# evanmayer/effex

Hardware: AMD Instinct MI355X
Metric: 2-ant FX correlator throughput (PFB+FFT+X, integrated) (higher is better)
Workload: dtype f32; 1 GPU; configs[1]: 2-antenna FX, num_samp=262144, ntaps=4, nchan=4096, 10000 integration frames per GPU per step; frames_per_gpu=10000, frames_total=10000, resident_frames=10000, num_samp=262144, nchan=4096, ntaps=4, n_ant=2, sample_definition=one complex sample per antenna stream, reduce_transport=none (single rank), library=effex_amd/csrc/libfxcorr.so

## Files before the change

effex_amd/csrc/fx_fused4096.h:

```cpp
#pragma once
#include "fx_math.h"

#if defined(__HIP_DEVICE_COMPILE__)
#define FXC_SCHED_FENCE() __builtin_amdgcn_sched_barrier(0)
#else
#define FXC_SCHED_FENCE() ((void)0)
#endif

namespace fxc {
namespace fused {

FX_HD cf lds_load(const cf* p) {
#if defined(__HIP_DEVICE_COMPILE__)
    typedef const volatile __attribute__((address_space(3))) unsigned long long* lds_u64_ptr;
    const unsigned long long u = *(lds_u64_ptr)(p);
    cf r;
    r.x = __uint_as_float((unsigned)(u & 0xffffffffull));
    r.y = __uint_as_float((unsigned)(u >> 32));
    return r;
#else
    return *p;
#endif
}

constexpr int kN = 4096;
constexpr int kT = 4;
constexpr int kThreads = 512;
constexpr int kRowPitch = 272;
constexpr int kRegion = 16 * kRowPitch;
constexpr int kAccPerThread = 8;
#ifndef FXC_FIR_GROUP
#define FXC_FIR_GROUP 4
#endif
constexpr int kFirGroup = FXC_FIR_GROUP;

constexpr int kLdsWin = 0;
constexpr int kLdsRegion = kLdsWin + kN * 16;
constexpr int kLdsTw2 = kLdsRegion + 2 * kRegion * 8;
constexpr int kLdsBytes = kLdsTw2 + 256 * 8;

struct State {
    cf h[4][16];
    cf tw1[16];
    cf acc[kAccPerThread];
};

template <int PH>
FX_HD void state_reset_history(State& s) {
#pragma unroll
    for (int d = 1; d < 4; ++d)
#pragma unroll
        for (int r = 0; r < 16; ++r) s.h[(PH + d) & 3][r] = mk(0.f, 0.f);
}

FX_HD void state_reset_all(State& s) {
    state_reset_history<0>(s);
#pragma unroll
    for (int q = 0; q < kAccPerThread; ++q) s.acc[q] = mk(0.f, 0.f);
}

struct RangeWalk {
    int c, i;
    int left;
    int row;
    int n_pts;
    int seg, seg_left;
    int seg_jump;
    int unit, in_row;
    int row_step;
    int row_off;
    bool rows_are_chunks;
    bool lead;
};

struct RangeSplit {
    int rounds, n_full, n_tail, rows_rounds, n_rows;
};

FX_HD RangeSplit range_split(int g, int n_chunks, int seg, int unit, bool rows_are_chunks) {
    RangeSplit r;
    r.rounds = n_chunks / (g * seg);
    r.n_full = r.rounds * g * seg;
    r.n_tail = n_chunks - r.n_full;
    r.rows_rounds = rows_are_chunks ? r.n_full : g * ((r.rounds * seg + unit - 1) / unit);
    r.n_rows = r.rows_rounds + r.n_tail + g;
    return r;
}

FX_HD RangeWalk range_walk_rounds(int b, int g, int n_chunks, int n_pts, int seg,
                                   int unit, bool rows_are_chunks) {
    const RangeSplit sp = range_split(g, n_chunks, seg, unit, rows_are_chunks);
    RangeWalk w;
    w.c = b * seg;
    w.i = 0;
    w.left = sp.rounds * seg * n_pts;
    w.n_pts = n_pts;
    w.seg = w.seg_left = seg;
    w.seg_jump = (g - 1) * seg;
    w.unit = rows_are_chunks ? 1 : unit;
    w.in_row = 0;
    w.rows_are_chunks = rows_are_chunks;
    w.row_off = 0;
    w.row_step = g;
    w.row = rows_are_chunks ? w.c : b;
    w.lead = false;
    return w;
}

FX_HD RangeWalk range_walk_tail(int b, int g, int n_chunks, int n_pts, int seg,
                                 int unit, bool rows_are_chunks) {
    const RangeSplit sp = range_split(g, n_chunks, seg, unit, rows_are_chunks);
    RangeWalk w;
    const int n_frames = sp.n_tail * n_pts;
    const int f0 = range_begin(b, n_frames, g);
    w.left = range_begin(b + 1, n_frames, g) - f0;
    w.c = sp.n_full + f0 / n_pts;
    w.i = f0 % n_pts;
    w.n_pts = n_pts;
    w.seg = 1;
    w.seg_left = 1;
    w.seg_jump = 0;
    w.unit = 1;
    w.in_row = 0;
    w.rows_are_chunks = true;
    w.row_off = sp.rows_rounds - sp.n_full;
    w.row_step = 0;
    w.lead = w.i != 0;
    w.row = w.lead ? sp.rows_rounds + sp.n_tail + b : w.c + w.row_off;
    return w;
}

FX_HD bool range_walk_row_ends(const RangeWalk& w) {
    return w.left == 1 || (w.i + 1 == w.n_pts && w.in_row + 1 == w.unit);
}

FX_HD void range_walk_prefetch(const RangeWalk& w, int& pc, int& pi) {
    pc = w.c;
    pi = w.i;
    if (w.left > 1 && ++pi == w.n_pts) {
        pi = 0;
        pc += 1 + (w.seg_left == 1 ? w.seg_jump : 0);
    }
}

FX_HD void range_walk_advance(RangeWalk& w, bool row_ended) {
    if (++w.i == w.n_pts) {
        w.i = 0;
        w.c += 1;
        if (--w.seg_left == 0) {
            w.c += w.seg_jump;
            w.seg_left = w.seg;
        }
        w.in_row += 1;
    }
    w.left -= 1;
    if (row_ended) {
        w.in_row = 0;
        w.row = w.rows_are_chunks ? w.c + w.row_off : w.row + w.row_step;
    }
}

FX_HD int sample_offset(int j, int r) { return (kN - 1) - j - 256 * r; }

template <int PH, int G = kFirGroup>
FX_HD void phase1_fir(const State& s, const f4* win, int tid, cf (&v)[16]) {
    const int j = tid & 255;
    const cf (&x0)[16] = s.h[PH];
    const cf (&x1)[16] = s.h[(PH + 3) & 3];
    const cf (&x2)[16] = s.h[(PH + 2) & 3];
    const cf (&x3)[16] = s.h[(PH + 1) & 3];
    constexpr int NG = 16 / G;
    f4 w[2][G];
#pragma unroll
    for (int q = 0; q < G; ++q) w[0][q] = win[q * 256 + j];
#pragma unroll
    for (int g = 0; g < NG; ++g) {
        if (g < NG - 1) {
#pragma unroll
            for (int q = 0; q < G; ++q) w[(g + 1) & 1][q] = win[(G * (g + 1) + q) * 256 + j];
        }
        FXC_SCHED_FENCE();
#pragma unroll
        for (int q = 0; q < G; ++q) {
            const int r = G * g + q;
            const f4 t = w[g & 1][q];
            cf a = cscale(x0[r], t.x);
            a = cfma(t.y, x1[r], a);
            a = cfma(t.z, x2[r], a);
            v[r] = cfma(t.w, x3[r], a);
        }
        FXC_SCHED_FENCE();
    }
}

FX_HD cf tw1_of(const cf (&pw2)[4], int k1) {
    cf w = mk(1.f, 0.f);
    bool have = false;
#pragma unroll
    for (int b = 0; b < 4; ++b) {
        if (k1 & (1 << b)) {
            w = have ? cmul(w, pw2[b]) : pw2[b];
            have = true;
        }
    }
    return w;
}

template <bool LEAN_TW = false>
FX_HD void phase1_finish_store(const State& s, cf (&v)[16], cf* region, int tid) {
    cf* mine = region + (tid >> 8) * kRegion + (tid & 255);
    cf pw2[4] = {s.tw1[1], s.tw1[2], s.tw1[4], s.tw1[8]};
#if defined(__HIP_DEVICE_COMPILE__)
    if (LEAN_TW) {
#pragma unroll
        for (int b = 0; b < 4; ++b) asm volatile("" : "+v"(pw2[b].x), "+v"(pw2[b].y));
    }
#endif
    dft16_b_stream(v, [&](int k1, cf val) {
        if (k1 > 0) val = cmul(val, LEAN_TW ? tw1_of(pw2, k1) : s.tw1[k1]);
        mine[k1 * kRowPitch] = val;
    });
}

FX_HD void state_load_twiddles(State& s, const cf* tw1_table, int tid) {
    const int j = tid & 255;
#pragma unroll
    for (int k1 = 0; k1 < 16; ++k1) s.tw1[k1] = tw1_table[k1 * 256 + j];
}

FX_HD cf* lane_row(cf* region, int tid) {
    const int l = tid & 63, wave = tid >> 6;
    const int ant = l >> 5, k1 = 2 * wave + ((l >> 4) & 1);
    return region + ant * kRegion + k1 * kRowPitch;
}

FX_HD void phase2_load(cf* region, int tid, cf (&v)[16]) {
    const cf* row = lane_row(region, tid);
    const int j0 = tid & 15;
#pragma unroll
    for (int j1 = 0; j1 < 16; ++j1) v[j1] = lds_load(row + j0 + 16 * j1);
}

FX_HD void phase2_twiddle(cf (&v)[16], const cf* tw2, int tid) {
    const int j0 = tid & 15;
    cf t[2][4];
#pragma unroll
    for (int q = 1; q < 4; ++q) t[0][q] = lds_load(tw2 + q * 16 + j0);
#pragma unroll
    for (int g = 0; g < 4; ++g) {
        if (g < 3) {
#pragma unroll
            for (int q = 0; q < 4; ++q) t[(g + 1) & 1][q] = lds_load(tw2 + (4 * (g + 1) + q) * 16 + j0);
        }
        FXC_SCHED_FENCE();
#pragma unroll
        for (int q = 0; q < 4; ++q) {
            const int q1 = 4 * g + q;
            if (q1 > 0) v[q1] = cmul(v[q1], t[g & 1][q]);
        }
        FXC_SCHED_FENCE();
    }
}

FX_HD void phase2_store(const cf (&v)[16], cf* region, int tid) {
    cf* row = lane_row(region, tid);
    const int j0 = tid & 15;
#pragma unroll
    for (int q1 = 0; q1 < 16; ++q1) row[q1 * 17 + j0] = v[q1];
}

FX_HD void phase3_load(cf* region, int tid, cf (&v)[16]) {
    const cf* row = lane_row(region, tid);
    const int q1 = tid & 15;
#pragma unroll
    for (int j0 = 0; j0 < 16; ++j0) v[j0] = lds_load(row + q1 * 17 + j0);
}

FX_HD void xacc(State& s, int q, cf a, cf b) { s.acc[q] = cmulc_acc(s.acc[q], a, b); }

FX_HD int bin_of(int tid, int q) {
    const int l = tid & 63, wave = tid >> 6;
    const int k1 = 2 * wave + ((l >> 4) & 1), q1 = l & 15, q2 = q + 8 * (l >> 5);
    return k1 + 16 * q1 + 256 * q2;
}

FX_HD int slot_of_bin(int k) {
    const int k1 = k & 15, q1 = (k >> 4) & 15, q2 = k >> 8;
    const int l = (q2 >> 3) * 32 + (k1 & 1) * 16 + q1;
    const int tid = (k1 >> 1) * 64 + l;
    return (q2 & 7) * kThreads + tid;
}

FX_HD int lane_specpos(int tid) {
    const int l = tid & 63, wave = tid >> 6;
    return (2 * wave + ((l >> 4) & 1)) * 16 + (l & 15);
}

FX_HD int specpos(int lane_l, int q2) { return (q2 >> 1) * 512 + 2 * lane_l + (q2 & 1); }
FX_HD int specpos_of_bin(int k) { return specpos((k & 15) * 16 + ((k >> 4) & 15), k >> 8); }

}
}
```

effex_amd/csrc/k_fused4096.h:

```cpp
#pragma once

namespace {

__device__ __forceinline__ void wave_sync() {
    __builtin_amdgcn_fence(__ATOMIC_RELEASE, "wavefront");
    __builtin_amdgcn_wave_barrier();
    __builtin_amdgcn_fence(__ATOMIC_ACQUIRE, "wavefront");
}

__device__ __forceinline__ void permlane32_swap(cf& a, cf& b) {
    auto rx = __builtin_amdgcn_permlane32_swap(__float_as_uint(a.x), __float_as_uint(b.x), false, false);
    auto ry = __builtin_amdgcn_permlane32_swap(__float_as_uint(a.y), __float_as_uint(b.y), false, false);
    a = fxc::mk(__uint_as_float(rx[0]), __uint_as_float(ry[0]));
    b = fxc::mk(__uint_as_float(rx[1]), __uint_as_float(ry[1]));
}

typedef unsigned v2u32 __attribute__((ext_vector_type(2)));
typedef unsigned v4u32 __attribute__((ext_vector_type(4)));
#ifndef FXC_LOAD_AUX_U8
#define FXC_LOAD_AUX_U8 2
#endif
#ifndef FXC_LOAD_AUX
#define FXC_LOAD_AUX 2
#endif
template <int R0, int CNT>
__device__ __forceinline__ void load_frame_part(cf (&xr)[16], const cf* chunk_base, unsigned chunk_bytes, unsigned voff,
                                                int64_t i) {
    __amdgpu_buffer_rsrc_t rs = __builtin_amdgcn_make_buffer_rsrc(const_cast<cf*>(chunk_base), 0, (int)chunk_bytes,
                                                                   0x00020000);
    const unsigned soff = (unsigned)(i * fxc::fused::kN * (int64_t)sizeof(cf));
#pragma unroll
    for (int r = R0; r < R0 + CNT; ++r) {
        const v2u32 d = __builtin_amdgcn_raw_buffer_load_b64(rs, voff, soff + (unsigned)(256 * (15 - r) * sizeof(cf)), FXC_LOAD_AUX);
        xr[r] = fxc::mk(__uint_as_float(d[0]), __uint_as_float(d[1]));
    }
}

template <int R0, int CNT>
__device__ __forceinline__ void load_frame_part_u8(cf (&xr)[16], const unsigned short* chunk_base,
                                                   unsigned chunk_bytes, unsigned voff, int64_t i) {
    __amdgpu_buffer_rsrc_t rs = __builtin_amdgcn_make_buffer_rsrc(const_cast<unsigned short*>(chunk_base), 0,
                                                                   (int)chunk_bytes, 0x00020000);
    const unsigned soff = (unsigned)(i * fxc::fused::kN * (int64_t)sizeof(unsigned short));
#pragma unroll
    for (int r = R0; r < R0 + CNT; ++r)
        xr[r].x = __uint_as_float(
            (unsigned)__builtin_amdgcn_raw_buffer_load_b16(rs, voff, soff + (unsigned)(256 * (15 - r) * sizeof(unsigned short)), FXC_LOAD_AUX_U8));
}

__device__ __forceinline__ void convert_frame_u8(cf (&h)[16], cf off) {
    const float k = 1.0f / 127.5f;
#pragma unroll
    for (int r = 0; r < 16; ++r) {
        const unsigned raw = __float_as_uint(h[r].x);
        h[r] = fxc::mk(fmaf((float)(raw & 0xFFu), k, off.x), fmaf((float)((raw >> 8) & 0xFFu), k, off.y));
    }
}

#ifndef FXC_ABL
#define FXC_ABL 0
#endif
#ifndef FXC_STAMPS
#define FXC_STAMPS 0
#endif
constexpr int kStampSegs = 12;
constexpr int kDckLdsBytes = 64;
constexpr int kAutoLdsBytes = fxc::fused::kAccPerThread * fxc::fused::kThreads * 4;
#if FXC_STAMPS
#define FXC_STAMP(k)                                                              \
    do {                                                                          \
        __builtin_amdgcn_sched_barrier(0);                                        \
        const unsigned long long t_now__ = __builtin_amdgcn_s_memtime();          \
        __builtin_amdgcn_s_waitcnt(0xC07F);                                       \
        seg[k] += t_now__ - t_prev;                                               \
        t_prev = t_now__;                                                         \
        __builtin_amdgcn_sched_barrier(0);                                        \
    } while (0)
#else
#define FXC_STAMP(k)
#endif
#if (FXC_ABL & 16)
#define FXC_PREFETCH(R0) ((void)0)
#else
#define FXC_PREFETCH(R0)                                                                                        \
    do {                                                                                                        \
        FXC_SCHED_FENCE();                                                                                      \
        if (U8)                                                                                                 \
            load_frame_part_u8<R0, 4>(nx, reinterpret_cast<const unsigned short*>(x) + (int64_t)pc * 2 * num_samp, \
                                      chunk_bytes, voff, nframe);                                               \
        else                                                                                                    \
            load_frame_part<R0, 4>(nx, nbase, chunk_bytes, voff, nframe);                                       \
        FXC_SCHED_FENCE();                                                                                      \
    } while (0)
#endif

struct U8State {
    cf off;
    bool have_next;
    bool rounds;
};

typedef unsigned v4u32_t __attribute__((ext_vector_type(4)));
constexpr int kDckStageVecs = 2 * fxc::fused::kThreads;

__device__ __forceinline__ void dck_fetch(const unsigned char* pair_base, int64_t num_samp, int64_t i, int tid, v4u32_t* stage) {
    typedef __attribute__((address_space(3))) v4u32_t* lptr_t;
    unsigned t = (unsigned)tid;
    asm volatile("" : "+v"(t));
    const unsigned lane_off = ((t >> 8) & 1u) * (unsigned)(2 * num_samp) + (t & 255u) * 16u;
    const unsigned char* base = pair_base + i * (fxc::fused::kThreads * 16);
    const unsigned lds_wave = __builtin_amdgcn_readfirstlane((unsigned)(size_t)(lptr_t)(stage + (t >> 6) * 128));
    unsigned m0_saved;
    asm volatile(
        "s_mov_b32 %[sv], m0\n\t"
        "s_mov_b32 m0, %[l0]\n\t"
        "s_nop 0\n\t"
        "global_load_lds_dwordx4 %[o0], %[base]\n\t"
        "s_add_u32 m0, %[l0], 0x400\n\t"
        "s_nop 0\n\t"
        "global_load_lds_dwordx4 %[o1], %[base]\n\t"
        "s_mov_b32 m0, %[sv]\n\t"
        : [sv] "=&s"(m0_saved)
        : [l0] "s"(lds_wave), [o0] "v"(lane_off), [o1] "v"(lane_off + 4096u), [base] "s"(base)
        : "memory", "scc");
}

__device__ __forceinline__ void dck_wait_prev() { asm volatile("s_waitcnt vmcnt(16)" ::: "memory"); }
__device__ __forceinline__ void dck_wait_own() { asm volatile("s_waitcnt vmcnt(4)" ::: "memory"); }

__device__ __forceinline__ void dck_clear(v4u32_t* stage, int tid) {
    unsigned z0;
    asm volatile("" : "+v"(tid));
    asm volatile("v_mov_b32 %0, 0" : "=v"(z0));
    const v4u32_t z = {z0, z0, z0, z0};
    stage[(tid >> 6) * 128 + (tid & 63)] = z;
    stage[(tid >> 6) * 128 + 64 + (tid & 63)] = z;
}

__device__ __forceinline__ void dck_add(const v4u32_t* stage, unsigned* acc, int tid) {
    asm volatile("" : "+v"(tid));
    unsigned si = 0u, sq = 0u;
#pragma unroll
    for (int h = 0; h < 2; ++h) {
        const v4u32_t w = stage[(tid >> 6) * 128 + h * 64 + (tid & 63)];
#pragma unroll
        for (int k = 0; k < 4; ++k) {
            si = __builtin_amdgcn_udot4(w[k], 0x00010001u, si, false);
            sq = __builtin_amdgcn_udot4(w[k], 0x01000100u, sq, false);
        }
    }
    acc[2 * tid] += si;
    acc[2 * tid + 1] += sq;
}

__device__ __forceinline__ cf dck_offset(unsigned* acc, unsigned* red, int tid, int64_t num_samp) {
    asm volatile("" : "+v"(tid));
    unsigned zero;
    asm volatile("v_mov_b32 %0, 0" : "=v"(zero));
    unsigned v[2] = {acc[2 * tid], acc[2 * tid + 1]};
    acc[2 * tid] = zero;
    acc[2 * tid + 1] = zero;
#pragma unroll
    for (int k = 0; k < 2; ++k) {
#pragma unroll
        for (int d = 32; d >= 1; d >>= 1) v[k] += __shfl_xor(v[k], d, 64);
    }
    __syncthreads();
    if ((tid & 63) == 0) {
        red[(tid >> 6) * 2] = v[0];
        red[(tid >> 6) * 2 + 1] = v[1];
    }
    __syncthreads();
    const int ant = (tid >> 8) & 1;
    unsigned long long ti = 0, tq = 0;
#pragma unroll
    for (int wv = 0; wv < 4; ++wv) {
        ti += red[(4 * ant + wv) * 2];
        tq += red[(4 * ant + wv) * 2 + 1];
    }
    asm volatile("" : "+s"(num_samp));
    const double mr = (double)ti / (double)num_samp, mi = (double)tq / (double)num_samp;
    return fxc::mk((float)(-mr / 127.5), (float)(-mi / 127.5));
}

#ifndef FXC_SPEC_STORE_AUX
#define FXC_SPEC_STORE_AUX 2
#endif
template <int PH, bool SPEC_OUT, bool U8, bool DCK, bool AUTOS>
__device__ __forceinline__ void fused_step(fxc::fused::State& s, float (&pw)[fxc::fused::kAccPerThread], float* pw_lds, U8State& u8, const cf* dc, const f4* win, cf* region,
                                           const cf* tw2, int tid, const cf* x, int64_t num_samp, unsigned chunk_bytes,
                                           unsigned voff, fxc::fused::RangeWalk& pos, cf* rows_raw, int hp, v4u32_t* dck_stage,
                                           unsigned* dck_acc, unsigned* dck_red,
                                           unsigned long long (&seg)[kStampSegs], unsigned long long& t_prev) {
    using namespace fxc::fused;
    const int64_t c = pos.c, i = pos.i, n_pts = pos.n_pts;
    FXC_STAMP(0);
    if (i == 0) {
        asm volatile("" ::: "memory");
        state_reset_history<PH>(s);
        if (U8) {
            if (DCK && u8.have_next) u8.off = dck_offset(dck_acc, dck_red, tid, num_samp);
            else u8.off = dc[c * 2 + __builtin_amdgcn_readfirstlane((tid >> 8) & 1)];
        }
    }
    const bool dck_next = DCK && u8.rounds && pos.left > n_pts - i;
    const unsigned char* dck_base = reinterpret_cast<const unsigned char*>(x) + (int64_t)(c + (dck_next ? 1 + pos.seg_jump : 0)) * 4 * num_samp;
    if (U8) convert_frame_u8(s.h[PH], u8.off);
    cf v[16];
    phase1_fir<PH, AUTOS ? 2 : kFirGroup>(s, win, tid, v);
    FXC_STAMP(2);
    int pc, nframe;
    range_walk_prefetch(pos, pc, nframe);
    const cf* nbase = x + (int64_t)pc * 2 * num_samp;
    cf (&nx)[16] = s.h[(PH + 1) & 3];
    FXC_PREFETCH(0);
    fxc::dft16_a(v);
    FXC_PREFETCH(4);
    FXC_STAMP(3);
#if !(FXC_ABL & 1)
    __syncthreads();
#endif
    FXC_STAMP(4);
#if !(FXC_ABL & 4)
    phase1_finish_store<AUTOS>(s, v, region, tid);
#endif
    FXC_STAMP(5);
#if !(FXC_ABL & 2)
    __syncthreads();
#endif
    if (DCK) {
        dck_wait_prev();
        dck_add(dck_stage, dck_acc, tid);
        dck_fetch(dck_base, num_samp, i, tid, dck_stage);
    }
    FXC_STAMP(6);
#if !(FXC_ABL & 4)
    phase2_load(region, tid, v);
#endif
    FXC_PREFETCH(8);
    fxc::dft16(v);
    FXC_STAMP(7);
    phase2_twiddle(v, tw2, tid);
    FXC_STAMP(8);
#if !(FXC_ABL & 8)
    wave_sync();
    phase2_store(v, region, tid);
    wave_sync();
#endif
    FXC_PREFETCH(12);
#if !(FXC_ABL & 8)
    phase3_load(region, tid, v);
#endif
    FXC_STAMP(9);
    fxc::dft16(v);
    if (SPEC_OUT) {
        const unsigned cu = (unsigned)c;
        const unsigned cr = hp == 1 ? cu : (hp == 2 ? cu >> 1 : (hp == 4 ? cu >> 2 : (unsigned)(((unsigned long long)cu * 0xAAAAAAABull) >> 33)));
        const int64_t row0 = ((int64_t)cr * n_pts + i) * (2 * hp) + 2 * (cu - cr * hp);
        __amdgpu_buffer_rsrc_t rs = __builtin_amdgcn_make_buffer_rsrc(rows_raw + row0 * kN, 0, (int)(2 * kN * (int64_t)sizeof(cf)), 0x00020000);
        const unsigned voff0 = (unsigned)(((tid >> 5) & 1) * kN + specpos(lane_specpos(tid), 0)) * (unsigned)sizeof(cf);
#pragma unroll
        for (int m = 0; m < 8; ++m) {
            v4u32 d = {__float_as_uint(v[2 * m].x), __float_as_uint(v[2 * m].y), __float_as_uint(v[2 * m + 1].x),
                       __float_as_uint(v[2 * m + 1].y)};
            __builtin_amdgcn_raw_buffer_store_b128(d, rs, voff0 + (unsigned)(m * 512 * sizeof(cf)), 0, FXC_SPEC_STORE_AUX);
        }
    } else {
#pragma unroll
        for (int q = 0; q < 8; ++q) {
            cf a = v[q], b = v[q + 8];
            permlane32_swap(a, b);
            xacc(s, q, a, b);
            if (AUTOS) {
                pw[q] = __builtin_fmaf(a.y, a.y, __builtin_fmaf(a.x, a.x, pw[q]));
                float* p1 = pw_lds + q * kThreads + tid;
                *p1 = __builtin_fmaf(b.y, b.y, __builtin_fmaf(b.x, b.x, *p1));
            }
        }
        FXC_STAMP(10);
    }
    if (DCK) {
        if (i + 1 == n_pts) {
            dck_wait_own();
            dck_add(dck_stage, dck_acc, tid);
            dck_clear(dck_stage, tid);
        }
        u8.have_next = dck_next;
    }
    const bool row_ends = !SPEC_OUT && range_walk_row_ends(pos);
    if (row_ends) {
        if (DCK) {
            __amdgpu_buffer_rsrc_t rs = __builtin_amdgcn_make_buffer_rsrc(rows_raw + (int64_t)pos.row * kN, 0, (int)(kN * (int64_t)sizeof(cf)), 0x00020000);
            unsigned t = (unsigned)tid;
            asm volatile("" : "+v"(t));
#pragma unroll
            for (int q = 0; q < kAccPerThread; ++q) {
                const v2u32 d = {__float_as_uint(s.acc[q].x), __float_as_uint(s.acc[q].y)};
                __builtin_amdgcn_raw_buffer_store_b64(d, rs, t * (unsigned)sizeof(cf), (unsigned)(q * kThreads * sizeof(cf)), 0);
                s.acc[q] = fxc::mk(0.f, 0.f);
            }
        } else {
            cf* row = rows_raw + (int64_t)pos.row * (AUTOS ? 3 : 1) * kN + tid;
#pragma unroll
            for (int q = 0; q < kAccPerThread; ++q) {
                row[q * kThreads] = s.acc[q];
                s.acc[q] = fxc::mk(0.f, 0.f);
                if (AUTOS) {
                    row[kN + q * kThreads] = fxc::mk(pw[q], 0.f);
                    row[2 * kN + q * kThreads] = fxc::mk(pw_lds[q * kThreads + tid], 0.f);
                    pw[q] = pw_lds[q * kThreads + tid] = 0.f;
                }
            }
        }
    }
    range_walk_advance(pos, row_ends);
}

template <bool SPEC_OUT, bool U8 = false, bool DCK = false, bool AUTOS = false>
__global__ __launch_bounds__(fxc::fused::kThreads, 2) void fx_fused4096_kernel(
    const cf* __restrict__ x, int64_t num_samp, int64_t n_pts, int64_t n_chunks, const f4* __restrict__ win_g,
    const cf* __restrict__ tw1_g, const cf* __restrict__ tw2_g, cf* __restrict__ rows_raw,
    unsigned long long* __restrict__ stamps, const cf* __restrict__ dc, int seg, int unit, int rows_are_chunks) {
    using namespace fxc::fused;
    extern __shared__ __attribute__((aligned(16))) unsigned char smem[];
    f4* win = reinterpret_cast<f4*>(smem + kLdsWin);
    cf* region = reinterpret_cast<cf*>(smem + kLdsRegion);
    cf* tw2 = reinterpret_cast<cf*>(smem + kLdsTw2);

    const int tid = threadIdx.x;
    const int ant = tid >> 8, j = tid & 255;
    for (int idx = tid; idx < kN; idx += kThreads) win[idx] = win_g[idx];
    if (tid < 256) tw2[tid] = tw2_g[tid];
    State s;
    state_load_twiddles(s, tw1_g, tid);
#pragma unroll
    for (int q = 0; q < kAccPerThread; ++q) s.acc[q] = fxc::mk(0.f, 0.f);
    static_assert(!AUTOS || (!SPEC_OUT && !U8), "autos: the complex64 F+X variant only");
    float pw[kAccPerThread];
    float* pw_lds = reinterpret_cast<float*>(smem + kLdsBytes);
#pragma unroll
    for (int q = 0; q < kAccPerThread; ++q) {
        pw[q] = 0.f;
        if (AUTOS) pw_lds[q * kThreads + tid] = 0.f;
    }
    __syncthreads();

    constexpr int64_t kSampleBytes = U8 ? sizeof(unsigned short) : sizeof(cf);
    const unsigned voff = (unsigned)((ant * num_samp + (255 - j)) * kSampleBytes);
    const unsigned chunk_bytes = (unsigned)(2 * num_samp * kSampleBytes);
    static_assert(!DCK || (U8 && !SPEC_OUT), "in-kernel DC removal: uint8 ingest only");
    U8State u8;
    u8.off = fxc::mk(0.f, 0.f);
    u8.have_next = u8.rounds = false;
    __shared__ v4u32_t dck_stage_mem[DCK ? kDckStageVecs : 1];
    __shared__ unsigned dck_acc_mem[DCK ? 2 * kThreads : 1];
    v4u32_t* dck_stage = dck_stage_mem;
    unsigned* dck_acc = dck_acc_mem;
    unsigned* dck_red = reinterpret_cast<unsigned*>(smem + kLdsBytes);
    if (DCK) {
        dck_acc[2 * tid] = dck_acc[2 * tid + 1] = 0u;
        dck_clear(dck_stage, tid);
    }
    unsigned long long seg_t[kStampSegs] = {0, 0, 0, 0, 0, 0, 0, 0, 0, 0, 0, 0};
    unsigned long long t_prev = 0;
    int64_t frames_done = 0;
#if FXC_STAMPS
    t_prev = __builtin_amdgcn_s_memtime();
#endif
#pragma unroll 1
    for (int part = 0; part < 2; ++part) {
        const int walk_unit = SPEC_OUT ? 1 : unit;
        int np_walk = (int)n_pts, seg_walk = seg, unit_walk = walk_unit;
        if (DCK) asm volatile("" : "+s"(np_walk), "+s"(seg_walk), "+s"(unit_walk));
        RangeWalk pos = part == 0 ? range_walk_rounds(blockIdx.x, gridDim.x, (int)n_chunks, np_walk, seg_walk, unit_walk, rows_are_chunks != 0)
                                  : range_walk_tail(blockIdx.x, gridDim.x, (int)n_chunks, np_walk, seg_walk, unit_walk, rows_are_chunks != 0);
        const int total = pos.left;
        if (!SPEC_OUT && part == 1 && (!pos.lead || total == 0)) {
            const RangeSplit sp = range_split(gridDim.x, (int)n_chunks, seg, walk_unit, rows_are_chunks != 0);
            int t_lead = tid;
            if (DCK) asm volatile("" : "+v"(t_lead));
            cf* lead_row = rows_raw + (int64_t)(sp.rows_rounds + sp.n_tail + blockIdx.x) * (AUTOS ? 3 : 1) * kN + t_lead;
#pragma unroll
            for (int q = 0; q < (AUTOS ? 3 : 1) * kAccPerThread; ++q) lead_row[q * kThreads] = fxc::mk(0.f, 0.f);
        }
        if (total == 0) continue;
        if (U8) u8.off = dc[(int64_t)pos.c * 2 + __builtin_amdgcn_readfirstlane(ant)];
        u8.have_next = false;
        u8.rounds = part == 0;
        const cf* cbase = reinterpret_cast<const cf*>(reinterpret_cast<const char*>(x) + (int64_t)pos.c * 2 * num_samp * kSampleBytes);
#pragma unroll
        for (int d = 1; d < 4; ++d) {
            if (pos.i - d >= 0) {
                if (U8) {
                    load_frame_part_u8<0, 16>(s.h[4 - d], reinterpret_cast<const unsigned short*>(cbase), chunk_bytes, voff, pos.i - d);
                    convert_frame_u8(s.h[4 - d], u8.off);
                } else {
                    load_frame_part<0, 16>(s.h[4 - d], cbase, chunk_bytes, voff, pos.i - d);
                }
            } else {
#pragma unroll
                for (int r = 0; r < 16; ++r) s.h[4 - d][r] = fxc::mk(0.f, 0.f);
            }
        }
        if (U8)
            load_frame_part_u8<0, 16>(s.h[0], reinterpret_cast<const unsigned short*>(cbase), chunk_bytes, voff, pos.i);
        else
            load_frame_part<0, 16>(s.h[0], cbase, chunk_bytes, voff, pos.i);
#pragma unroll 1
        for (int g = 0; g < total; g += 4) {
            fused_step<0, SPEC_OUT, U8, DCK, AUTOS>(s, pw, pw_lds, u8, dc, win, region, tw2, tid, x, num_samp, chunk_bytes, voff, pos, rows_raw, SPEC_OUT ? unit : 0, dck_stage, dck_acc, dck_red, seg_t, t_prev);
            if (g + 1 < total)
                fused_step<1, SPEC_OUT, U8, DCK, AUTOS>(s, pw, pw_lds, u8, dc, win, region, tw2, tid, x, num_samp, chunk_bytes, voff, pos, rows_raw, SPEC_OUT ? unit : 0, dck_stage, dck_acc, dck_red, seg_t, t_prev);
            if (g + 2 < total)
                fused_step<2, SPEC_OUT, U8, DCK, AUTOS>(s, pw, pw_lds, u8, dc, win, region, tw2, tid, x, num_samp, chunk_bytes, voff, pos, rows_raw, SPEC_OUT ? unit : 0, dck_stage, dck_acc, dck_red, seg_t, t_prev);
            if (g + 3 < total)
                fused_step<3, SPEC_OUT, U8, DCK, AUTOS>(s, pw, pw_lds, u8, dc, win, region, tw2, tid, x, num_samp, chunk_bytes, voff, pos, rows_raw, SPEC_OUT ? unit : 0, dck_stage, dck_acc, dck_red, seg_t, t_prev);
        }
        frames_done += total;
    }
#if FXC_STAMPS
    if (stamps && (tid & 63) == 0) {
        unsigned long long* dst = stamps + ((int64_t)blockIdx.x * (kThreads / 64) + (tid >> 6)) * kStampSegs;
        for (int k = 0; k < kStampSegs; ++k) dst[k] = seg_t[k];
        dst[kStampSegs - 1] = (unsigned long long)frames_done;
    }
#else
    (void)stamps;
    (void)frames_done;
#endif
}

}
```

Baseline: 305,000 Msamples/s.

## Split LDS exchange into real/imag planes with permuted branch mapping and addtid stores

Changes the shared-memory transpose buffers from interleaved complex rows to separate real and imaginary float planes with new pitches. Stores now use ds_write_addtid_b32 with an M0 base and compile-time offsets. Threads are permuted to a new branch mapping so each lane's writes are contiguous and conflict-free, with the window and twiddle loads reindexed to match. The aim is fewer LDS bank conflicts and less address arithmetic in the FFT exchange phases. In exchange it relies on inline asm and M0 handling, and the index permutations must stay consistent across the FIR, load and store phases.

```diff
diff --git a/effex_amd/csrc/fx_fused4096.h b/effex_amd/csrc/fx_fused4096.h
--- a/effex_amd/csrc/fx_fused4096.h
+++ b/effex_amd/csrc/fx_fused4096.h
@@ -26,18 +26,77 @@
 constexpr int kN = 4096;
 constexpr int kT = 4;
 constexpr int kThreads = 512;
-constexpr int kRowPitch = 272;
-constexpr int kRegion = 16 * kRowPitch;
+constexpr int kPlaneRow = 288;
+constexpr int kPlane = 16 * kPlaneRow;
+constexpr int kAntPlanes = 2 * kPlane;
+constexpr int kRegionBytes = 2 * kAntPlanes * 4;
 constexpr int kAccPerThread = 8;
 #ifndef FXC_FIR_GROUP
 #define FXC_FIR_GROUP 4
 #endif
 constexpr int kFirGroup = FXC_FIR_GROUP;
 
-constexpr int kLdsWin = 0;
-constexpr int kLdsRegion = kLdsWin + kN * 16;
-constexpr int kLdsTw2 = kLdsRegion + 2 * kRegion * 8;
+constexpr int kLdsRegion = 0;
+constexpr int kLdsWin = kLdsRegion + kRegionBytes;
+constexpr int kLdsTw2 = kLdsWin + kN * 16;
 constexpr int kLdsBytes = kLdsTw2 + 256 * 8;
+
+FX_HD int branch_of_thread(int t) {
+    const int l = t & 63, wv = (t >> 6) & 3;
+    return ((l >> 1) & 15) + 16 * ((l & 1) | ((l >> 5) << 1) | (wv << 2));
+}
+FX_HD int thread_of_branch(int j) { return ((j >> 4) & 1) | ((j & 15) << 1) | (j & 0xE0); }
+
+struct LaneStore {
+#if defined(__HIP_DEVICE_COMPILE__)
+    unsigned m0;
+#else
+    float* at;
+#endif
+};
+
+FX_HD LaneStore lane_store_begin(cf* region, int base_dw, int lane) {
+    LaneStore ls;
+#if defined(__HIP_DEVICE_COMPILE__)
+    typedef __attribute__((address_space(3))) cf* lptr_t;
+    (void)lane;
+    ls.m0 = __builtin_amdgcn_readfirstlane((unsigned)(size_t)(lptr_t)region + 4u * (unsigned)base_dw);
+    asm volatile("s_nop 0" : : "{m0}"(ls.m0));
+#else
+    ls.at = reinterpret_cast<float*>(region) + base_dw + lane;
+#endif
+    return ls;
+}
+
+template <int DW>
+FX_HD void lane_store(const LaneStore& ls, float val) {
+    static_assert(DW >= 0 && 4 * DW < 65536, "16-bit immediate");
+#if defined(__HIP_DEVICE_COMPILE__)
+    asm volatile("ds_write_addtid_b32 %0 offset:%1" : : "v"(val), "n"(4 * DW), "{m0}"(ls.m0));
+#else
+    ls.at[DW] = val;
+#endif
+}
+
+FX_HD void lane_store_end() {
+#if defined(__HIP_DEVICE_COMPILE__)
+    asm volatile("s_waitcnt lgkmcnt(0)" : : : "memory");
+#endif
+}
+
+template <int K>
+struct KConst { static constexpr int value = K; };
+template <class Sink>
+FX_HD void dft16_b_stream_ct(cf (&v)[16], Sink&& sink) {
+    dft4(v[0], v[1], v[2], v[3]);
+    sink(KConst<0>{}, v[0]); sink(KConst<4>{}, v[1]); sink(KConst<8>{}, v[2]); sink(KConst<12>{}, v[3]);
+    dft4_scaled_c_bd(v[4], v[5], v[6], v[7]);
+    sink(KConst<1>{}, v[4]); sink(KConst<5>{}, v[5]); sink(KConst<9>{}, v[6]); sink(KConst<13>{}, v[7]);
+    dft4_bd_scaled(v[8], v[9], v[10], v[11]);
+    sink(KConst<2>{}, v[8]); sink(KConst<6>{}, v[9]); sink(KConst<10>{}, v[10]); sink(KConst<14>{}, v[11]);
+    dft4_scaled_c_bd(v[12], v[13], v[14], v[15]);
+    sink(KConst<3>{}, v[12]); sink(KConst<7>{}, v[13]); sink(KConst<11>{}, v[14]); sink(KConst<15>{}, v[15]);
+}
 
 struct State {
     cf h[4][16];
@@ -163,8 +222,8 @@
 FX_HD int sample_offset(int j, int r) { return (kN - 1) - j - 256 * r; }
 
 template <int PH, int G = kFirGroup>
-FX_HD void phase1_fir(const State& s, const f4* win, int tid, cf (&v)[16]) {
-    const int j = tid & 255;
+FX_HD void phase1_fir_col(const State& s, const f4* win, int col, cf (&v)[16]) {
+    const int j = col;
     const cf (&x0)[16] = s.h[PH];
     const cf (&x1)[16] = s.h[(PH + 3) & 3];
     const cf (&x2)[16] = s.h[(PH + 2) & 3];
@@ -193,6 +252,11 @@
     }
 }
 
+template <int PH, int G = kFirGroup>
+FX_HD void phase1_fir(const State& s, const f4* win, int tid, cf (&v)[16]) {
+    phase1_fir_col<PH, G>(s, win, tid & 255, v);
+}
+
 FX_HD cf tw1_of(const cf (&pw2)[4], int k1) {
     cf w = mk(1.f, 0.f);
     bool have = false;
@@ -208,7 +272,8 @@
 
 template <bool LEAN_TW = false>
 FX_HD void phase1_finish_store(const State& s, cf (&v)[16], cf* region, int tid) {
-    cf* mine = region + (tid >> 8) * kRegion + (tid & 255);
+    const int t = thread_of_branch(tid & 255);
+    const LaneStore ls = lane_store_begin(region, (tid >> 8) * kAntPlanes + (t & 0xC0), t & 63);
     cf pw2[4] = {s.tw1[1], s.tw1[2], s.tw1[4], s.tw1[8]};
 #if defined(__HIP_DEVICE_COMPILE__)
     if (LEAN_TW) {
@@ -216,10 +281,13 @@
         for (int b = 0; b < 4; ++b) asm volatile("" : "+v"(pw2[b].x), "+v"(pw2[b].y));
     }
 #endif
-    dft16_b_stream(v, [&](int k1, cf val) {
+    dft16_b_stream_ct(v, [&](auto k, cf val) {
+        constexpr int k1 = decltype(k)::value;
         if (k1 > 0) val = cmul(val, LEAN_TW ? tw1_of(pw2, k1) : s.tw1[k1]);
-        mine[k1 * kRowPitch] = val;
+        lane_store<k1 * kPlaneRow>(ls, val.x);
+        lane_store<kPlane + k1 * kPlaneRow>(ls, val.y);
     });
+    lane_store_end();
 }
 
 FX_HD void state_load_twiddles(State& s, const cf* tw1_table, int tid) {
@@ -228,17 +296,17 @@
     for (int k1 = 0; k1 < 16; ++k1) s.tw1[k1] = tw1_table[k1 * 256 + j];
 }
 
-FX_HD cf* lane_row(cf* region, int tid) {
+FX_HD void phase2_load(cf* region, int tid, cf (&v)[16]) {
     const int l = tid & 63, wave = tid >> 6;
-    const int ant = l >> 5, k1 = 2 * wave + ((l >> 4) & 1);
-    return region + ant * kRegion + k1 * kRowPitch;
-}
-
-FX_HD void phase2_load(cf* region, int tid, cf (&v)[16]) {
-    const cf* row = lane_row(region, tid);
-    const int j0 = tid & 15;
-#pragma unroll
-    for (int j1 = 0; j1 < 16; ++j1) v[j1] = lds_load(row + j0 + 16 * j1);
+    const int ant = l >> 5, k1 = 2 * wave + ((l >> 4) & 1), j0 = l & 15;
+    const float* row = reinterpret_cast<const float*>(region) + ant * kAntPlanes + k1 * kPlaneRow + 2 * j0;
+#pragma unroll
+    for (int u = 0; u < 8; ++u) {
+        const cf re = lds_load(reinterpret_cast<const cf*>(row + 32 * u));
+        const cf im = lds_load(reinterpret_cast<const cf*>(row + kPlane + 32 * u));
+        v[2 * u] = mk(re.x, im.x);
+        v[2 * u + 1] = mk(re.y, im.y);
+    }
 }
 
 FX_HD void phase2_twiddle(cf (&v)[16], const cf* tw2, int tid) {
@@ -262,18 +330,32 @@
     }
 }
 
+constexpr int kStripeHi = kPlane + 32;
+constexpr int stripe_of(int q1) { return (q1 >> 3) * kStripeHi + (q1 & 7) * 66; }
+
+template <int Q1>
+FX_HD void phase2_store_from(const LaneStore& ls, const cf (&v)[16]) {
+    lane_store<stripe_of(Q1)>(ls, v[Q1].x);
+    lane_store<stripe_of(Q1) + kAntPlanes>(ls, v[Q1].y);
+    if constexpr (Q1 < 15) phase2_store_from<Q1 + 1>(ls, v);
+}
+
 FX_HD void phase2_store(const cf (&v)[16], cf* region, int tid) {
-    cf* row = lane_row(region, tid);
-    const int j0 = tid & 15;
-#pragma unroll
-    for (int q1 = 0; q1 < 16; ++q1) row[q1 * 17 + j0] = v[q1];
+    const LaneStore ls = lane_store_begin(region, (tid >> 6) * 2 * kPlaneRow, tid & 63);
+    phase2_store_from<0>(ls, v);
+    lane_store_end();
 }
 
 FX_HD void phase3_load(cf* region, int tid, cf (&v)[16]) {
-    const cf* row = lane_row(region, tid);
-    const int q1 = tid & 15;
-#pragma unroll
-    for (int j0 = 0; j0 < 16; ++j0) v[j0] = lds_load(row + q1 * 17 + j0);
+    const int l = tid & 63, wave = tid >> 6, q1 = l & 15;
+    const float* row = reinterpret_cast<const float*>(region) + wave * 2 * kPlaneRow + stripe_of(q1) + (l >> 4) * 16;
+#pragma unroll
+    for (int u = 0; u < 8; ++u) {
+        const cf re = lds_load(reinterpret_cast<const cf*>(row + 2 * u));
+        const cf im = lds_load(reinterpret_cast<const cf*>(row + kAntPlanes + 2 * u));
+        v[2 * u] = mk(re.x, im.x);
+        v[2 * u + 1] = mk(re.y, im.y);
+    }
 }
 
 FX_HD void xacc(State& s, int q, cf a, cf b) { s.acc[q] = cmulc_acc(s.acc[q], a, b); }
diff --git a/effex_amd/csrc/k_fused4096.h b/effex_amd/csrc/k_fused4096.h
--- a/effex_amd/csrc/k_fused4096.h
+++ b/effex_amd/csrc/k_fused4096.h
@@ -207,7 +207,7 @@
     const unsigned char* dck_base = reinterpret_cast<const unsigned char*>(x) + (int64_t)(c + (dck_next ? 1 + pos.seg_jump : 0)) * 4 * num_samp;
     if (U8) convert_frame_u8(s.h[PH], u8.off);
     cf v[16];
-    phase1_fir<PH, AUTOS ? 2 : kFirGroup>(s, win, tid, v);
+    phase1_fir_col<PH, AUTOS ? 2 : kFirGroup>(s, win, tid & 255, v);
     FXC_STAMP(2);
     int pc, nframe;
     range_walk_prefetch(pos, pc, nframe);
@@ -222,7 +222,7 @@
 #endif
     FXC_STAMP(4);
 #if !(FXC_ABL & 4)
-    phase1_finish_store<AUTOS>(s, v, region, tid);
+    phase1_finish_store<AUTOS>(s, v, region, (tid & ~255) | branch_of_thread(tid & 255));
 #endif
     FXC_STAMP(5);
 #if !(FXC_ABL & 2)
@@ -328,11 +328,11 @@
     cf* tw2 = reinterpret_cast<cf*>(smem + kLdsTw2);
 
     const int tid = threadIdx.x;
-    const int ant = tid >> 8, j = tid & 255;
-    for (int idx = tid; idx < kN; idx += kThreads) win[idx] = win_g[idx];
+    const int ant = tid >> 8, j = branch_of_thread(tid & 255);
+    for (int idx = tid; idx < kN; idx += kThreads) win[idx] = win_g[(idx & ~255) | branch_of_thread(idx & 255)];
     if (tid < 256) tw2[tid] = tw2_g[tid];
     State s;
-    state_load_twiddles(s, tw1_g, tid);
+    state_load_twiddles(s, tw1_g, (ant << 8) | j);
 #pragma unroll
     for (int q = 0; q < kAccPerThread; ++q) s.acc[q] = fxc::mk(0.f, 0.f);
     static_assert(!AUTOS || (!SPEC_OUT && !U8), "autos: the complex64 F+X variant only");
```

New measurement: 315,600 Msamples/s, median of 6. 3.5% higher.
